# abelxiaoxing/ImageClassification

Hardware: AMD Instinct MI355X
Metric: images/sec (whole node) ResNet-50 bf16 224^2 training (higher is better)
Workload: dtype bf16; 1 GPU; resnet50 train step, synthetic 3x224x224, batch 256/GPU, AdamW, label smoothing 0.1, 1000 classes (BASELINE configs[1]); global_batch=256, parallelism=dp1

## Files before the change

imageclassification_amd/csrc/capi.hip:

```cpp
#include "../../include/icamd.h"
#include "common.h"
#include "icamd_internal.h"
#include <cstdlib>
#include <string.h>

int icamd_bn_finalize_launch(const float* part, int nrows, int C, double count, const float* gamma, const float* beta,
                             float* running_mean, float* running_var, float momentum, float eps, float* mean,
                             float* invstd, float* scale, float* shift, double* chunks, hipStream_t s);
int icamd_bn_eval_coeffs_launch(int C, const float* gamma, const float* beta, const float* rm, const float* rv, float eps,
                                float* scale, float* shift, hipStream_t s);
int icamd_bn_apply_launch(const bf16_t* y, const float* scale, const float* shift, const bf16_t* residual, bf16_t* out,
                          unsigned char* maskbits, long long numel, int C, int relu, hipStream_t s,
                          const float* res_scale = nullptr, const float* res_shift = nullptr);
int icamd_bn_bwd_rows_per_block(long long rows, int C);
int icamd_bn_bwd_launch(const bf16_t* dout, const bf16_t* act, const bf16_t* y, const float* mean, const float* invstd,
                        const float* scale, const float* shift, float* dgamma, float* dbeta, bf16_t* dy, bf16_t* gout,
                        const unsigned char* maskbits, long long rows, int C, int relu, int accumulate, float* part,
                        double* chunks, float* c1c2, hipStream_t s, const unsigned char* pool_idx = nullptr,
                        int pool_ih = 0, int pool_iw = 0);
int icamd_bn_bwd_dual_launch(const bf16_t* dout, const unsigned char* maskbits, const bf16_t* yA, const float* meanA,
                             const float* invstdA, const float* scaleA, float* dgammaA, float* dbetaA, bf16_t* dyA,
                             const bf16_t* yB, const float* meanB, const float* invstdB, const float* scaleB, float* dgammaB,
                             float* dbetaB, bf16_t* dyB, long long rows, int C, int accumulate, float* partA, double* chunksA,
                             float* cA, float* partB, double* chunksB, float* cB, hipStream_t s);
// ... 105 lines not shown
int icamd_se_bn_apply_launch(const bf16_t* y, const float* scale, const float* shift, const float* gate, const bf16_t* residual,
                             const float* res_scale, const float* res_shift, bf16_t* out, unsigned char* maskbits, int N, int HW,
                             int C, int relu, hipStream_t s);
size_t icamd_se_bn_bwd_bytes(int N, int HW, int C);
int icamd_se_bn_bwd_launch(const bf16_t* dout, const unsigned char* maskbits, const bf16_t* y, const float* mean,
                           const float* invstd, const float* gamma, const float* beta, const float* ysum, const float* sv,
                           const float* h, const float* e, const float* w1, const float* w2, float* dgamma, float* dbeta,
                           float* dw1, float* db1, float* dw2, float* db2, bf16_t* dy, int N, int HW, int C, int rd,
                           int accumulate, void* workspace, hipStream_t s);


#include <vector>
namespace {
enum ProfClass { PC_IGEMM_FWD = 0, PC_IGEMM_DGRAD, PC_WGRAD, PC_BN_FINALIZE, PC_BN_APPLY, PC_BN_BWD, PC_POOL, PC_PACK,
                 PC_LOSS, PC_OPTIM, PC_MISC, PC_ATTN_FWD, PC_ATTN_BWD, PC_LN_FWD, PC_LN_BWD, PC_ELEMWISE, PC_DWCONV, PC_FUSED_BWD, PC_FUSED_FWD, PC_COUNT };
struct ProfRec { int cls; hipEvent_t a, b; double bytes, flops; };
bool g_prof_on = false;
std::vector<ProfRec> g_prof_recs;
std::vector<hipEvent_t> g_prof_pool;
hipEvent_t prof_event() {
  if (!g_prof_pool.empty()) { hipEvent_t e = g_prof_pool.back(); g_prof_pool.pop_back(); return e; }
  hipEvent_t e; (void)hipEventCreate(&e); return e;
}
struct ProfScope {
  int cls; hipStream_t s; hipEvent_t a; bool on; double bytes = 0.0, flops = 0.0;
  ProfScope(int c, void* stream) : cls(c), s((hipStream_t)stream), on(g_prof_on) {
    if (on) { a = prof_event(); (void)hipEventRecord(a, s); }
  }
  void work(double b, double f = 0.0) { bytes = b; flops = f; }
  ~ProfScope() {
    if (on) { hipEvent_t b = prof_event(); (void)hipEventRecord(b, s); g_prof_recs.push_back({cls, a, b, bytes, flops}); }
  }
};
struct ConvWork { double in, out, w, flops; };
static ConvWork conv_work(const icamd_conv_desc* d) {
  ConvWork c = {0, 0, 0, 0};
  if (d == nullptr) return c;
  c.in = 2.0 * d->N * d->IH * d->IW * d->Cin;
  c.out = 2.0 * d->N * d->OH * d->OW * d->Cout;
  c.w = (double)d->Cout * d->KH * d->KW * d->Cin;
  c.flops = 2.0 * d->N * d->OH * d->OW * c.w;
  return c;
}
}

namespace {
// ... 14 lines not shown
}

extern "C" {

int icamd_abi_version(void) { return 6; }

int icamd_prof_enable(int on) { g_prof_on = on != 0; return ICAMD_OK; }
int icamd_prof_classes(void) { return PC_COUNT; }
int icamd_prof_collect(double* ms, long long* calls, double* bytes, double* flops, int n) {
  if (ms == nullptr || calls == nullptr || n < PC_COUNT) return ICAMD_ERR_BAD_ARG;
  for (auto& r : g_prof_recs) {
    (void)hipEventSynchronize(r.b);
    float t = 0.f;
    (void)hipEventElapsedTime(&t, r.a, r.b);
    ms[r.cls] += (double)t;
    calls[r.cls] += 1;
    if (bytes != nullptr) bytes[r.cls] += r.bytes;
    if (flops != nullptr) flops[r.cls] += r.flops;
    g_prof_pool.push_back(r.a);
    g_prof_pool.push_back(r.b);
  }
  g_prof_recs.clear();
  return ICAMD_OK;
}

int icamd_conv2d_stats_rows(const icamd_conv_desc* d) {
  if (!conv_desc_ok(d)) return 0;
  const long long M = (long long)d->N * d->OH * d->OW;
  return (int)((M + 127) / 128);
}

// ... 306 lines not shown
  int rc;
  if (dbias == nullptr && icamd_wgrad_halo_wanted(d->KH, d->KW, d->stride, d->pad, d->OH, d->OW, d->Cin, d->Cout, p.M)) {
    icamd_wgrad_halo_plan(p.M, p.Cin, p.Cout, &p.S, &p.rows_per_split);
    rc = icamd_wgrad_halo_launch(p, (hipStream_t)stream);
  } else {
    icamd_wgrad_plan(p.M, p.Cout, p.Ktot, &p.S, &p.rows_per_split);
    if (dbias != nullptr) p.bias_slab = p.slab + (size_t)p.S * p.Cout * p.Ktot;
    rc = icamd_wgrad_launch(p, (hipStream_t)stream);
  }
  if (rc) return rc;
  rc = icamd_slab_reduce_launch(p.slab, dw, (long long)p.Cout * p.Ktot, p.S, accumulate, (hipStream_t)stream);
  if (rc || dbias == nullptr) return rc;
  return icamd_slab_reduce_launch(p.bias_slab, dbias, (long long)p.Cout, p.S, accumulate, (hipStream_t)stream);
}

static bool gconv_ok(const icamd_conv_desc* d, int groups) {
  if (!conv_desc_ok(d) || groups <= 0) return false;
  if (d->KH != 3 || d->KW != 3 || d->pad != 1 || d->Cin != d->Cout) return false;
  return icamd_gconv3x3_ok(d->N, d->IH, d->IW, d->OH, d->OW, d->Cin, groups, d->stride);
}
static GConvParams gconv_params(const icamd_conv_desc* d, int groups) {
  GConvParams p;
  memset(&p, 0, sizeof(p));
  p.N = d->N; p.IH = d->IH; p.IW = d->IW; p.OH = d->OH; p.OW = d->OW; p.C = d->Cin; p.groups = groups; p.stride = d->stride;
  return p;
}
static void gconv_work(ProfScope& prof, const icamd_conv_desc* d, int groups, double filter_bytes_per_element) {
  if (d == nullptr || groups <= 0) return;
  const double wel = 9.0 * d->Cout * (d->Cin / groups);
  prof.work(2.0 * d->N * d->IH * d->IW * d->Cin + 2.0 * d->N * d->OH * d->OW * d->Cout + filter_bytes_per_element * wel,
// ... 1035 lines not shown
```

imageclassification_amd/csrc/conv_wgrad.hip:

```cpp
#include "common.h"
#include "icamd_internal.h"
#include <stdlib.h>

namespace {

constexpr int BKR = 64;

template <int W>
__device__ __forceinline__ int tr_swz(int row) {
  if constexpr (W >= 128) return (row & 3) | (((row >> 3) & 1) << 2);
  else return ((row >> 1) & 1) | (((row >> 3) & 1) << 1);
}

__device__ __forceinline__ bf16x8 tr_read_pair(const unsigned char* p0, const unsigned char* p1) {
  bf16x4 a = __builtin_amdgcn_ds_read_tr16_b64_v4i16((bf16x4 __attribute__((address_space(3)))*)p0);
  bf16x4 b = __builtin_amdgcn_ds_read_tr16_b64_v4i16((bf16x4 __attribute__((address_space(3)))*)p1);
  return bf16x8{a[0], a[1], a[2], a[3], b[0], b[1], b[2], b[3]};
}

__device__ __forceinline__ void wgrad_block_order(const WgradParams& p, unsigned int& tile, int& split) {
  const unsigned int nt = (unsigned)(p.ntiles_k * p.ntiles_c);
  if (p.xcd_chunk) {
    const unsigned int nblk = gridDim.x, xcd = blockIdx.x & 7u, idx = blockIdx.x >> 3;
    const unsigned int q = nblk >> 3, r = nblk & 7u;
// ... 4 lines not shown
  }
  const unsigned int grp = blockIdx.x / (8u * nt);
  const unsigned int rem = blockIdx.x - grp * 8u * nt;
  const unsigned int ns = min(8u, (unsigned)p.S - grp * 8u);
  tile = rem / ns;
  split = (int)(grp * 8u + (rem - tile * ns));
}

#ifndef ICAMD_WGRAD_STAGES
#define ICAMD_WGRAD_STAGES 1
#endif
#ifndef ICAMD_WGRAD_WAVES_PER_SIMD
#define ICAMD_WGRAD_WAVES_PER_SIMD 3
#endif

template <int BMK, int BNC>
__global__ __launch_bounds__(256, (ICAMD_WGRAD_STAGES == 1 ? ICAMD_WGRAD_WAVES_PER_SIMD : 2)) void conv_wgrad_kernel(const WgradParams p) {
  constexpr int NSTAGE = ICAMD_WGRAD_STAGES;
  constexpr int X_BYTES = BKR * BMK * 2;
  constexpr int Y_BYTES = BKR * BNC * 2;
  constexpr int STAGE_BYTES = X_BYTES + Y_BYTES;
  constexpr int XROWB = BMK * 2, YROWB = BNC * 2;
  constexpr int XCPR = BMK / 8, YCPR = BNC / 8;
  constexpr int XRPI = 64 / XCPR, YRPI = 64 / YCPR;
  constexpr int XJ = BMK / 32, YJ = BNC / 32;
  constexpr int KR = BMK / 32, CR = BNC / 32;
  __shared__ __attribute__((aligned(16))) unsigned char smem[NSTAGE * STAGE_BYTES];

  const int tid = threadIdx.x, lane = tid & 63, wave = tid >> 6;
  const int wk = wave & 1, wc = wave >> 1;

  unsigned int tile;
  int split;
  wgrad_block_order(p, tile, split);
  const int tile_c = (int)(tile % (unsigned)p.ntiles_c);
  const int tile_k = (int)(tile / (unsigned)p.ntiles_c);
  const int k0 = tile_k * BMK, c0 = tile_c * BNC;
  const int m_begin = split * p.rows_per_split;
  const int m_end = min(p.M, m_begin + p.rows_per_split);

  const bf16_t* __restrict__ x = p.x;
  const bf16_t* __restrict__ dy = p.dy;
  const bf16_t* zero = (const bf16_t*)icamd_zero_page;

  int x_row[XJ], x_dh[XJ], x_dw[XJ], x_ci[XJ];
#pragma unroll
  for (int j = 0; j < XJ; ++j) {
    const int row = (wave * XJ + j) * XRPI + lane / XCPR;
    const int pc = lane % XCPR;
// ... 508 lines not shown
      *(f32x4*)(slab + (long long)co * p.Ktot + kk) = acc[jj][ii];
    }
  if (do_bias && (lane >> 4) == 0) {
#pragma unroll
    for (int j = 0; j < 2; ++j) p.bias_slab[(long long)split * p.Cout + c0 + wc * 64 + wr * 32 + j * 16 + (lane & 15)] = bacc[j][0];
  }
}

#ifndef ICAMD_SLAB_NT
#define ICAMD_SLAB_NT 1
#endif
__device__ __forceinline__ f32x4 slab_ld(const f32x4* p) {
  if constexpr (ICAMD_SLAB_NT != 0) return __builtin_nontemporal_load(p);
  else return *p;
}
template <int OUTS>
__global__ __launch_bounds__(256) void slab_reduce_kernel(const float* __restrict__ slab, float* __restrict__ out,
                                                          long long n4, int S, int accumulate, int stem7_mask) {
  constexpr int LANES = 256 / OUTS;
  __shared__ f32x4 red[256];
  const int o = threadIdx.x % OUTS, l = threadIdx.x / OUTS;
  const long long i = (long long)blockIdx.x * OUTS + o;
  f32x4 a0 = {0.f, 0.f, 0.f, 0.f}, a1 = a0, a2 = a0, a3 = a0;
  if (i < n4) {
    const f32x4* p = (const f32x4*)slab + i;
    int k = l;
    for (; k + 3 * LANES < S; k += 4 * LANES) {
      a0 += slab_ld(p + (long long)k * n4);
      a1 += slab_ld(p + (long long)(k + LANES) * n4);
      a2 += slab_ld(p + (long long)(k + 2 * LANES) * n4);
      a3 += slab_ld(p + (long long)(k + 3 * LANES) * n4);
    }
    for (; k < S; k += LANES) a0 += slab_ld(p + (long long)k * n4);
  }
  red[threadIdx.x] = (a0 + a1) + (a2 + a3);
  __syncthreads();
  if (l == 0 && i < n4) {
// ... 311 lines not shown
  if (bmk == 256 && bnc == 256) return launch_ring<256, 256, 2, 4, 4, 2>(p, stream);
  if (bmk == 256 && bnc == 128) return launch_ring<256, 128, 2, 2, 3, 2>(p, stream);
  if (bmk == 128 && bnc == 256) return launch_ring<128, 256, 1, 4, 3, 2>(p, stream);
  if (bmk == 256 && bnc == 64) return launch_ring<256, 64, 4, 1, 3, 2>(p, stream);
  if (bmk == 64 && bnc == 256) return launch_ring<64, 256, 1, 4, 3, 2>(p, stream);
  if (bmk == 128 && bnc == 128) return launch_ring<128, 128, 2, 2, 3, 3>(p, stream);
  if (bmk == 128 && bnc == 64) return launch_ring<128, 64, 2, 2, 3, 3>(p, stream);
  if (bmk == 64 && bnc == 128) return launch_ring<64, 128, 2, 2, 3, 3>(p, stream);
  return launch_ring<64, 64, 2, 2, 3, 3>(p, stream);
}

int icamd_slab_reduce_launch(const float* slab, float* out, long long n, int S, int accumulate, hipStream_t stream,
                             int stem7_mask) {
  if (n % 4 != 0) return ICAMD_ERR_BAD_ARG;
  const long long n4 = n / 4;
  if (n4 >= 64 * 1024) {
    hipLaunchKernelGGL(slab_reduce_kernel<64>, dim3((unsigned)((n4 + 63) / 64)), dim3(256), 0, stream, slab, out, n4, S,
                       accumulate, stem7_mask);
  } else {
    hipLaunchKernelGGL(slab_reduce_kernel<16>, dim3((unsigned)((n4 + 15) / 16)), dim3(256), 0, stream, slab, out, n4, S,
                       accumulate, stem7_mask);
  }
  return icamd_launch_status();
}
```

imageclassification_amd/csrc/icamd_internal.h:

```cpp
#pragma once
#include "common.h"

#define ICAMD_MAX_TAPS 56

struct IgemmParams {
  const bf16_t* in;
  const bf16_t* wt;
  bf16_t* out;
  const bf16_t* addend;
  const unsigned char* addend_bits;
  int addend_sub2;
  const float* bias;
  float* stats;
  const bf16_t* bnb_y;
  const bf16_t* bnb_mask;
  const float *bnb_mean, *bnb_invstd, *bnb_scale, *bnb_shift;
  int bnb_relu;
  int relu;
  bf16_t* gelu_out;
  int gelu_inplace;
  const bf16_t* gelu_z;
  int N, IH, IW, Cin;
  int OH, OW, Cout;
  int P, Q, M;
// ... 193 lines not shown
  int S, rows_per_split;
  int ntiles_k, ntiles_c;
  int pointwise;
  int xcd_chunk;
  int stem7;
  FastDiv divHW, divW, divCin, divKW;
};
int icamd_wgrad_launch(WgradParams& p, hipStream_t stream);
void icamd_wgrad_plan(int M, int Cout, int Ktot, int* S, int* rows_per_split);
void icamd_wgrad_tile(long long M, int Ktot, int Cout, int* bmk, int* bnc);
bool icamd_wgrad_halo_wanted(int KH, int KW, int stride, int pad, int H, int W, int Cin, int Cout, long long M);
void icamd_wgrad_halo_plan(int M, int Cin, int Cout, int* S, int* rows_per_split);
int icamd_wgrad_halo_launch(WgradParams& p, hipStream_t stream);
int icamd_slab_reduce_launch(const float* slab, float* out, long long n, int S, int accumulate, hipStream_t stream,
                             int stem7_mask = 0);
```

imageclassification_amd/hip.py:

```python
import ctypes
import os
from ctypes import POINTER, Structure, c_double, c_float, c_int, c_longlong, c_size_t, c_void_p

import torch

_HERE = os.path.dirname(os.path.abspath(__file__))
LIB_PATH = os.path.join(_HERE, "csrc", "libicamd.so")

ABI_VERSION = 6
ERRORS = {1: "ICAMD_ERR_BAD_ARG", 2: "ICAMD_ERR_UNSUPPORTED", 3: "ICAMD_ERR_WORKSPACE", 4: "ICAMD_ERR_LAUNCH"}


class IcamdError(RuntimeError):
    pass


class BnBwdFuse(Structure):
    _fields_ = [("y", c_void_p), ("mask_src", c_void_p), ("mean", c_void_p), ("invstd", c_void_p), ("scale", c_void_p),
                ("shift", c_void_p), ("partials", c_void_p), ("relu", c_int)]


class ImageDesc(Structure):
    _fields_ = [("src_offset", ctypes.c_int64), ("src_h", c_int), ("src_w", c_int), ("crop_top", c_int), ("crop_left", c_int),
                ("crop_h", c_int), ("crop_w", c_int), ("hflip", c_int), ("vflip", c_int), ("jitter_order", c_int * 3),
# ... 37 lines not shown
    "icamd_conv2d_dgrad_sub2": (c_int, [POINTER(ConvDesc), _P, _P, _P, _P, _P]),
    "icamd_conv2d_dgrad_stats_rows": (c_int, [POINTER(ConvDesc)]),
    "icamd_conv2d_dgrad_bnbwd": (c_int, [POINTER(ConvDesc), _P, _P, _P, _P, POINTER(BnBwdFuse), _P]),
    "icamd_conv2d_dgrad_bnred_supported": (c_int, [POINTER(ConvDesc)]),
    "icamd_conv2d_dgrad_bnred": (c_int, [POINTER(ConvDesc), _P, _P, _P, _P, _P, c_int, _P, _P, _P, _P]),
    "icamd_bn_bwd_from_gy_partials": (c_int, [_P, c_int, _P, _P, _P, _P, _P, _P, _P, _P, c_longlong, c_int, c_int, _P, c_size_t, _P]),
    "icamd_bn_apply_conv1x1_fused_supported": (c_int, [POINTER(ConvDesc)]),
    "icamd_bn_apply_conv1x1_fused": (c_int, [POINTER(ConvDesc), _P, _P, _P, _P, _P, _P, _P, _P, _P, _P, _P, _P]),
    "icamd_conv1x1_bn_bwd_fused_supported": (c_int, [POINTER(ConvDesc)]),
    "icamd_conv1x1_bn_bwd_fused_workspace_bytes": (c_size_t, [POINTER(ConvDesc)]),
    "icamd_conv1x1_bn_bwd_fused": (c_int, [POINTER(ConvDesc), _P, c_int, _P, _P, _P, _P, _P, _P, _P, _P, _P, _P, _P, c_int, _P, c_size_t,
                                           _P, c_size_t, _P]),
    "icamd_conv2d_wgrad_workspace_bytes": (c_size_t, [POINTER(ConvDesc)]),
    "icamd_conv2d_wgrad": (c_int, [POINTER(ConvDesc), _P, _P, _P, c_int, _P, c_size_t, _P]),
    "icamd_conv2d_wgrad_bias": (c_int, [POINTER(ConvDesc), _P, _P, _P, _P, c_int, _P, c_size_t, _P]),
    "icamd_gconv3x3_supported": (c_int, [POINTER(ConvDesc), c_int]),
    "icamd_gconv3x3_fwd": (c_int, [POINTER(ConvDesc), c_int, _P, _P, _P, _P, _P]),
    "icamd_gconv3x3_fwd_act": (c_int, [POINTER(ConvDesc), c_int, _P, _P, _P, _P, c_int, _P]),
    "icamd_gconv3x3_dgrad": (c_int, [POINTER(ConvDesc), c_int, _P, _P, _P, _P]),
    "icamd_gconv3x3_wgrad_workspace_bytes": (c_size_t, [POINTER(ConvDesc), c_int]),
    "icamd_gconv3x3_wgrad": (c_int, [POINTER(ConvDesc), c_int, _P, _P, _P, c_int, _P, c_size_t, _P]),
    "icamd_avgpool2x2_fwd": (c_int, [_P, _P, c_int, c_int, c_int, c_int, _P]),
    "icamd_avgpool2x2_bwd": (c_int, [_P, _P, _P, c_int, c_int, c_int, c_int, _P]),
    "icamd_conv3x3_thin_supported": (c_int, [POINTER(ConvDesc)]),
    "icamd_conv3x3_thin_stats_rows": (c_int, [POINTER(ConvDesc)]),
    "icamd_conv3x3_thin_fwd": (c_int, [POINTER(ConvDesc), _P, _P, _P, _P, _P, c_int, _P]),
    "icamd_conv3x3_thin_dgrad": (c_int, [POINTER(ConvDesc), _P, _P, _P, _P]),
    "icamd_conv3x3_thin_wgrad_workspace_bytes": (c_size_t, [POINTER(ConvDesc)]),
    "icamd_conv3x3_thin_wgrad": (c_int, [POINTER(ConvDesc), _P, _P, _P, c_int, _P, c_size_t, _P]),
    "icamd_filter_transpose": (c_int, [_P, _P, _P, _P, c_int, _P]),
# ... 157 lines not shown
```

imageclassification_amd/nets.py:

```python
import ctypes
import itertools
import math
import os
from collections import OrderedDict
from types import SimpleNamespace

import torch

from . import hip
from .checkpoint import PicklableModel
from .streams import side_lane

BN_EPS = 1e-5
_FUSED_BNBWD = os.environ.get("ICAMD_FUSED_BNBWD", "0") == "1"
_WGRAD_STREAM = os.environ.get("ICAMD_WGRAD_STREAM", "1") != "0"
_DUAL_BNBWD = os.environ.get("ICAMD_DUAL_BNBWD", "1") != "0"
_SUB2_SHORTCUT = os.environ.get("ICAMD_SUB2_SHORTCUT", "1") != "0"
_FUSED_POOL_BWD = os.environ.get("ICAMD_FUSED_POOL_BWD", "1") != "0"
_STEM_THIN_DEFAULT = {"fwd": True, "dgrad": True, "wgrad": False}
_STEM_THIN_ENV = os.environ.get("ICAMD_STEM_THIN", "1")
_STEM_THIN = {op: (_STEM_THIN_ENV == "2" or (_STEM_THIN_ENV != "0" and on)) for op, on in _STEM_THIN_DEFAULT.items()}
BN_MOMENTUM = 0.1

ARCHS = {
    "resnet18": ("basic", [2, 2, 2, 2], 1, 64),
    "resnet34": ("basic", [3, 4, 6, 3], 1, 64),
    "resnet50": ("bottleneck", [3, 4, 6, 3], 1, 64),
    "resnet101": ("bottleneck", [3, 4, 23, 3], 1, 64),
    "resnet152": ("bottleneck", [3, 8, 36, 3], 1, 64),
    "wide_resnet50_2": ("bottleneck", [3, 4, 6, 3], 1, 128),
    "wide_resnet101_2": ("bottleneck", [3, 4, 23, 3], 1, 128),
    "resnext50_32x4d": ("bottleneck", [3, 4, 6, 3], 32, 4),
# ... 109 lines not shown

class _Conv:

    def __init__(self, name, cin, cout, k, stride, pad, cin_p=None, cout_p=None, bias=False, k_p=None, groups=1):
        self.name = name
        self.groups = groups
        self.cin, self.cout, self.k, self.stride, self.pad = cin, cout, k, stride, pad
        self.cin_p = cin_p or cin
        self.cout_p = cout_p or cout
        self.k_p = k_p or k
        self.has_bias = bias
        self.w = None
        self.b = None
        self.wt_offset = None
        self.descs = {}
        self.thin = False
        self.stem7 = False

    def desc(self, N, IH, IW):
        key = (N, IH, IW)
        d = self.descs.get(key)
        if d is None:
            d = hip.conv_desc(N, IH, IW, self.cin_p, self.cout_p, self.k, self.k, self.stride, self.pad)
            self.descs[key] = d
        return d


class _BN:
    def __init__(self, name, c):
        self.name, self.c = name, c
# ... 728 lines not shown
        return ws["logits"]

    def __call__(self, x_nchw):
        ws = self.pack(x_nchw.to(self.device, dtype=torch.float32).contiguous())
        logits = self.forward_packed(ws)
        return logits[:, : self.num_classes]

    def backward_packed(self, ws, accumulate=False):
        if _FUSED_BNBWD:
            if self.se:
                raise hip.IcamdError("ICAMD_FUSED_BNBWD=1 has no squeeze-and-excitation backward")
            if self.deep:
                raise hip.IcamdError("ICAMD_FUSED_BNBWD=1 has no average-pool shortcut backward")
            return self._backward_packed_fused(ws, accumulate)
        run = self._backward_begin(ws, accumulate, _WGRAD_STREAM and self.wgrad_side_stream)
        bufs = self._grad_buffers(ws)
        dout, other, run.T, run.DA = (b.data_ptr() for b in bufs[:4])
        run.ypool = itertools.cycle([b.data_ptr() for b in bufs[4:]])
        self._bwd_classifier(run, dout)
        fused_rows = 0
        for bi in range(len(self.blocks) - 1, -1, -1):
            dy, dy2, shortcut_done = self._bwd_last_bn(run, bi, dout, fused_rows)
            dy = self._bwd_inner_convs(run, bi, dy)
            fused_rows = self._bwd_conv1_shortcut(run, bi, dy, dy2, shortcut_done, dout, other)
            if run.hook:
                run.hook(self.blocks[bi]["convs"][0].w.offset, None, run.lane.events())
            dout, other = other, dout
        self._bwd_stem(run, dout, self._next_y(run), _FUSED_POOL_BWD)
        if run.hook:
            run.hook(0, None, run.lane.events())
        run.lane.join()

    def _backward_begin(self, ws, accumulate, side):
        lane = side_lane(self, "ICAMD_WGRAD_STREAM", True)
        lane.begin(side)
        return SimpleNamespace(ws=ws, N=ws["N"], acc=int(bool(accumulate)), lane=lane, s=lane.main.cuda_stream,
                               hook=self.grad_ready_hook, wsp=ws["wgrad_ws"].data_ptr(), wsb=ws["wgrad_ws_bytes"],
                               bws=ws["bnb_ws"].data_ptr(), bwb=ws["bnb_ws_bytes"])

    def _next_y(self, run):
        y = next(run.ypool)
        run.lane.before_write(y)
        return y

    def _side_wgrad(self, run, conv, d, x, dy):
        run.lane.launch(lambda st: self._wgrad(conv, d, x, dy, run.acc, run.wsp, run.wsb, st), reads=(dy,))

    def _bn_bwd(self, run, bn, dout, act, y, dy, gout, relu, maskbits=None):
        mean, invstd, scale, shift = self._stats(bn)
        c = bn.c
        hip.check(self.lib.icamd_bn_bwd(dout, act, y.data_ptr(), mean, invstd, scale, shift, self._gf(bn.weight),
                                        self._gf(bn.bias), dy, gout, maskbits, y.numel() // c, c, int(relu), run.acc, run.bws,
                                        run.bwb, run.s), bn.name + " bwd")

    def _fused_conv_bn(self, run, conv, bn, d, partials, nrows, g, y, x, dx, bn_ws, bn_ws_bytes):
        lib, ws = self.lib, run.ws
        mean, invstd, scale, _ = self._stats(bn)
        need = lib.icamd_conv1x1_bn_bwd_fused_workspace_bytes(ctypes.byref(d))
        fws = ws.get("fused_ws")
        if fws is None or fws.numel() < need:
            fws = ws["fused_ws"] = torch.empty(need, dtype=torch.uint8, device=self.device)
# ... 8 lines not shown
        dfc = self.fc.desc(N, 1, 1)
        self._side_wgrad(run, self.fc, dfc, ws["pooled"].data_ptr(), dl)
        hip.check(lib.icamd_colsum(dl, N, self.ncls_p, self.ncls_p, self._gf(self.fc.b), run.acc, s), "fc bias grad")
        self._dgrad(self.fc, dfc, dl, ws["dpooled"].data_ptr(), None, None, s)
        if run.hook:
            run.hook(self.fc.w.offset, self.n_params, run.lane.events())
        fh, fw = ws["final_hw"]
        hip.check(lib.icamd_avgpool_bwd(ws["dpooled"].data_ptr(), dout, N, fh * fw, self.feat_dim, s), "avgpool bwd")

    def _bwd_last_bn(self, run, bi, dout, fused_rows):
        lib, ws, N = self.lib, run.ws, run.N
        blk, b = self.blocks[bi], ws["blocks"][bi]
        conv3, bn3, y3 = blk["convs"][-1], blk["bns"][-1], b["y"][-1]
        down = "down_conv" in blk
        mask = b["mask"].data_ptr()
        dy = self._next_y(run)
        dy2, shortcut_done = None, False
        d3 = conv3.desc(N, *b["hw"][-1])
        if "se" in blk:
            se = blk["se"]
            mean, invstd, _, _ = self._stats(bn3)
            hip.check(lib.icamd_se_bn_bwd(dout, mask, y3.data_ptr(), mean, invstd, self._pf(bn3.weight), self._pf(bn3.bias),
                                          b["se_ysum"].data_ptr(), b["se_s"].data_ptr(), b["se_h"].data_ptr(),
                                          b["se_e"].data_ptr(), self._pf(se.w1), self._pf(se.w2), self._gf(bn3.weight),
                                          self._gf(bn3.bias), self._gf(se.w1), self._gf(se.b1), self._gf(se.w2), self._gf(se.b2),
                                          dy, N, d3.OH * d3.OW, se.c, se.rd, run.acc, ws["se_ws"].data_ptr(), ws["se_ws_bytes"],
                                          run.s), se.name + " + " + bn3.name + " bwd")
            return dy, None, False
        if (self.block == "bottleneck" and fused_rows > 0 and lib.icamd_conv1x1_bn_bwd_fused_supported(ctypes.byref(d3))):
            self._fused_conv_bn(run, conv3, bn3, d3, ws["bnb_part"].data_ptr(), fused_rows, dout, y3, b["a"][-2].data_ptr(), run.DA,
                                ws["bna_ws"].data_ptr(), ws["bna_ws_bytes"])
            dy = None
            if down:
                dc = blk["down_conv"]
                ddc = dc.desc(N, *b.get("short_hw", b["in_hw"]))
                if dc.stride == 1 and lib.icamd_conv1x1_bn_bwd_fused_supported(ctypes.byref(ddc)):
                    self._fused_conv_bn(run, dc, blk["down_bn"], ddc, None, 0, dout, b["yd"], b.get("xp", b["in"]).data_ptr(),
                                        run.T, run.bws, run.bwb)
                    shortcut_done = True
                else:
                    dy2 = self._next_y(run)
                    self._bn_bwd(run, blk["down_bn"], dout, None, b["yd"], dy2, None, False)
        elif down and _DUAL_BNBWD:
            dy2 = self._next_y(run)
            bnB = blk["down_bn"]
            meanA, invstdA, scaleA, _ = self._stats(bn3)
            meanB, invstdB, scaleB, _ = self._stats(bnB)
            c = bn3.c
            hip.check(lib.icamd_bn_bwd_dual(dout, mask, y3.data_ptr(), meanA, invstdA, scaleA, self._gf(bn3.weight),
                                            self._gf(bn3.bias), dy, b["yd"].data_ptr(), meanB, invstdB, scaleB,
                                            self._gf(bnB.weight), self._gf(bnB.bias), dy2, y3.numel() // c, c, run.acc, run.bws,
                                            ws["bnb_ws2"].data_ptr(), run.bwb, run.s), bn3.name + " + shortcut bwd")
        elif fused_rows:
            mean, invstd, scale, _ = self._stats(bn3)
            c = bn3.c
            hip.check(lib.icamd_bn_bwd_from_gy_partials(ws["bnb_part"].data_ptr(), fused_rows, dout, y3.data_ptr(), mean, invstd,
                                                        scale, self._gf(bn3.weight), self._gf(bn3.bias), dy, y3.numel() // c, c,
                                                        run.acc, ws["bna_ws"].data_ptr(), ws["bna_ws_bytes"], run.s),
                      bn3.name + " bwd (apply, sums from the data gradient)")
        else:
            self._bn_bwd(run, bn3, dout, None, y3, dy, None, True, mask)
        return dy, dy2, shortcut_done

    def _bwd_inner_convs(self, run, bi, dy):
        blk, b = self.blocks[bi], run.ws["blocks"][bi]
        convs, bns = blk["convs"], blk["bns"]
        for i in range(len(convs) - 1, 0, -1):
            if dy is not None:
                d = convs[i].desc(run.N, *b["hw"][i])
                self._side_wgrad(run, convs[i], d, b["a"][i - 1].data_ptr(), dy)
                self._dgrad(convs[i], d, dy, run.DA, None, None, run.s)
            dy = self._next_y(run)
            self._bn_bwd(run, bns[i - 1], run.DA, None, b["y"][i - 1], dy, None, True)
        return dy

    def _prev_takes_g(self, N, bi, h, w):
        if bi == 0 or self.block != "bottleneck":
            return False
        pblk = self.blocks[bi - 1]
        if "se" in pblk:
            return False
        if "down_conv" not in pblk:
            return True
        dp3 = pblk["convs"][-1].desc(N, h, w)
        return bool(self.lib.icamd_conv1x1_bn_bwd_fused_supported(ctypes.byref(dp3)))

    def _bwd_conv1_shortcut(self, run, bi, dy, dy2, shortcut_done, dout, other):
        lib, ws, N, s = self.lib, run.ws, run.N, run.s
        blk, b = self.blocks[bi], ws["blocks"][bi]
        conv1 = blk["convs"][0]
        h, w = b["in_hw"]
        xin = b["in"].data_ptr()
        d1 = conv1.desc(N, h, w)
        self._side_wgrad(run, conv1, d1, xin, dy)
        if blk.get("pool"):
            dc = blk["down_conv"]
            ddc = dc.desc(N, *b["short_hw"])
            if not shortcut_done:
                if dy2 is None:
                    dy2 = self._next_y(run)
                    self._bn_bwd(run, blk["down_bn"], dout, None, b["yd"], dy2, None, True, b["mask"].data_ptr())
                self._side_wgrad(run, dc, ddc, b["xp"].data_ptr(), dy2)
                self._dgrad(dc, ddc, dy2, run.T, None, None, s)
            self._dgrad(conv1, d1, dy, run.DA, None, None, s)
            hip.check(lib.icamd_avgpool2x2_bwd(run.T, run.DA, other, N, h, w, dc.cin_p, s), blk["name"] + " shortcut pool bwd")
            return 0
        if shortcut_done:
            self._dgrad(conv1, d1, dy, other, run.T, None, s)
            return 0
        if "down_conv" not in blk:
            addend, bits, on_even_grid = dout, b["mask"].data_ptr(), 0
        else:
            dc = blk["down_conv"]
            ddc = dc.desc(N, h, w)
            if dy2 is None:
                dy2 = self._next_y(run)
                self._bn_bwd(run, blk["down_bn"], dout, None, b["yd"], dy2, None, True, b["mask"].data_ptr())
            self._side_wgrad(run, dc, ddc, xin, dy2)
            if not (_SUB2_SHORTCUT and dc.k == 1 and dc.stride == 2 and dc.pad == 0):
                self._dgrad(dc, ddc, dy2, run.T, None, None, s)
                self._dgrad(conv1, d1, dy, other, run.T, None, s)
                return 0
            key = ("sub2", N, ddc.OH, ddc.OW)
            deven = dc.descs.get(key)
            if deven is None:
                deven = dc.descs[key] = hip.conv_desc(N, ddc.OH, ddc.OW, dc.cin_p, dc.cout_p, 1, 1, 1, 0)
            self._dgrad(dc, deven, dy2, run.T, None, None, s)
            addend, bits, on_even_grid = run.T, None, 1
        if self._prev_takes_g(N, bi, h, w) and lib.icamd_conv2d_dgrad_bnred_supported(ctypes.byref(d1)):
            pb = ws["blocks"][bi - 1]
            hip.check(lib.icamd_conv2d_dgrad_bnred(ctypes.byref(d1), dy, self._wt(conv1), other, addend, bits, on_even_grid,
# ... 110 lines not shown
```

include/icamd.h:

```cpp
#ifndef ICAMD_H
#define ICAMD_H
#include <stddef.h>
#include <stdint.h>

#ifdef __cplusplus
extern "C" {
#endif

#define ICAMD_OK 0
#define ICAMD_ERR_BAD_ARG 1
#define ICAMD_ERR_UNSUPPORTED 2
#define ICAMD_ERR_WORKSPACE 3
#define ICAMD_ERR_LAUNCH 4

int icamd_abi_version(void);

typedef struct icamd_conv_desc {
  int N, IH, IW, Cin;
  int OH, OW, Cout;
  int KH, KW, stride, pad;
} icamd_conv_desc;

int icamd_conv2d_stats_rows(const icamd_conv_desc* d);

// ... 19 lines not shown
  const void* y;
  const void* mask_src;
  const float *mean, *invstd, *scale, *shift;
  float* partials;
  int relu;
} icamd_bn_bwd_fuse;
int icamd_conv2d_dgrad_stats_rows(const icamd_conv_desc* d);
int icamd_conv2d_dgrad_bnbwd(const icamd_conv_desc* d, const void* dy, const void* w_t, void* g, const void* addend,
                             const icamd_bn_bwd_fuse* f, void* stream);

size_t icamd_conv2d_wgrad_workspace_bytes(const icamd_conv_desc* d);
int icamd_conv2d_wgrad(const icamd_conv_desc* d, const void* x, const void* dy, float* dw, int accumulate,
                       void* workspace, size_t workspace_bytes, void* stream);
int icamd_conv2d_wgrad_bias(const icamd_conv_desc* d, const void* x, const void* dy, float* dw, float* dbias,
                            int accumulate, void* workspace, size_t workspace_bytes, void* stream);

int icamd_gconv3x3_supported(const icamd_conv_desc* d, int groups);
int icamd_gconv3x3_fwd(const icamd_conv_desc* d, int groups, const void* x, const void* w, void* y, float* stats, void* stream);
int icamd_gconv3x3_fwd_act(const icamd_conv_desc* d, int groups, const void* x, const void* w, void* y, const float* bias, int relu,
                           void* stream);
int icamd_gconv3x3_dgrad(const icamd_conv_desc* d, int groups, const void* dy, const void* w, void* dx, void* stream);
size_t icamd_gconv3x3_wgrad_workspace_bytes(const icamd_conv_desc* d, int groups);
int icamd_gconv3x3_wgrad(const icamd_conv_desc* d, int groups, const void* x, const void* dy, float* dw, int accumulate,
                         void* workspace, size_t workspace_bytes, void* stream);

int icamd_filter_transpose(const void* src_base, void* dst_base, const int64_t* descs, const int32_t* jobs, int njobs,
                           void* stream);
int icamd_filter_transpose_tiled(const void* src_base, void* dst_base, const int64_t* descs, const int32_t* jobs,
                                 int njobs, void* stream);

// ... 247 lines not shown
```

Baseline: 14720 images/sec.

## Batch pointwise 1x1 weight-gradient convs into grouped wgrad and slab-reduce launches

Adds a grouped weight-gradient path that queues up to twelve 1x1 stride-1 convs with equal row counts and runs them as one multi-job GEMM kernel plus one grouped slab-reduce kernel on the side stream. Queued convs write their output gradients into dedicated held buffers so the data stays valid until the grouped launch. This targets launch overhead and under-filled grids from many small wgrad GEMMs. In exchange it uses extra memory for the held buffers and a larger workspace, and it delays gradient readiness, which changes when the hooks fire and how the work overlaps.

```diff
diff --git a/imageclassification_amd/csrc/capi.hip b/imageclassification_amd/csrc/capi.hip
--- a/imageclassification_amd/csrc/capi.hip
+++ b/imageclassification_amd/csrc/capi.hip
@@ -143,7 +143,7 @@
 namespace {
 enum ProfClass { PC_IGEMM_FWD = 0, PC_IGEMM_DGRAD, PC_WGRAD, PC_BN_FINALIZE, PC_BN_APPLY, PC_BN_BWD, PC_POOL, PC_PACK,
                  PC_LOSS, PC_OPTIM, PC_MISC, PC_ATTN_FWD, PC_ATTN_BWD, PC_LN_FWD, PC_LN_BWD, PC_ELEMWISE, PC_DWCONV, PC_FUSED_BWD, PC_FUSED_FWD, PC_COUNT };
-struct ProfRec { int cls; hipEvent_t a, b; double bytes, flops; };
+struct ProfRec { int cls; hipEvent_t a, b; double bytes, flops; int calls; };
 bool g_prof_on = false;
 std::vector<ProfRec> g_prof_recs;
 std::vector<hipEvent_t> g_prof_pool;
@@ -153,12 +153,13 @@
 }
 struct ProfScope {
   int cls; hipStream_t s; hipEvent_t a; bool on; double bytes = 0.0, flops = 0.0;
+  int calls = 1;
   ProfScope(int c, void* stream) : cls(c), s((hipStream_t)stream), on(g_prof_on) {
     if (on) { a = prof_event(); (void)hipEventRecord(a, s); }
   }
   void work(double b, double f = 0.0) { bytes = b; flops = f; }
   ~ProfScope() {
-    if (on) { hipEvent_t b = prof_event(); (void)hipEventRecord(b, s); g_prof_recs.push_back({cls, a, b, bytes, flops}); }
+    if (on) { hipEvent_t b = prof_event(); (void)hipEventRecord(b, s); g_prof_recs.push_back({cls, a, b, bytes, flops, calls}); }
   }
 };
 struct ConvWork { double in, out, w, flops; };
@@ -203,7 +204,7 @@
     float t = 0.f;
     (void)hipEventElapsedTime(&t, r.a, r.b);
     ms[r.cls] += (double)t;
-    calls[r.cls] += 1;
+    calls[r.cls] += r.calls;
     if (bytes != nullptr) bytes[r.cls] += r.bytes;
     if (flops != nullptr) flops[r.cls] += r.flops;
     g_prof_pool.push_back(r.a);
@@ -540,6 +541,62 @@
   return icamd_slab_reduce_launch(p.bias_slab, dbias, (long long)p.Cout, p.S, accumulate, (hipStream_t)stream);
 }
 
+int icamd_conv2d_wgrad_group_supported(const icamd_conv_desc* d) {
+  if (!conv_desc_ok(d)) return 0;
+  return icamd_wgrad_group_wanted(d->KH, d->KW, d->stride, d->pad, (long long)d->N * d->OH * d->OW, d->Cin, d->Cout) ? 1 : 0;
+}
+
+int icamd_conv2d_wgrad_group_plan(int n, const icamd_conv_desc* const* d, int* S, int* rows_per_split, unsigned int* first_block) {
+  if (n < 1 || n > ICAMD_WGRAD_GROUP_MAX || d == nullptr || S == nullptr || rows_per_split == nullptr || first_block == nullptr)
+    return ICAMD_ERR_BAD_ARG;
+  int M[ICAMD_WGRAD_GROUP_MAX], ci[ICAMD_WGRAD_GROUP_MAX], co[ICAMD_WGRAD_GROUP_MAX];
+  for (int j = 0; j < n; ++j) {
+    if (!icamd_conv2d_wgrad_group_supported(d[j])) return ICAMD_ERR_UNSUPPORTED;
+    M[j] = d[j]->N * d[j]->OH * d[j]->OW; ci[j] = d[j]->Cin; co[j] = d[j]->Cout;
+  }
+  icamd_wgrad_group_plan(n, M, ci, co, S, rows_per_split, first_block);
+  return ICAMD_OK;
+}
+
+size_t icamd_conv2d_wgrad_group_workspace_bytes(int n, const icamd_conv_desc* const* d) {
+  int S[ICAMD_WGRAD_GROUP_MAX], rows[ICAMD_WGRAD_GROUP_MAX];
+  unsigned int first[ICAMD_WGRAD_GROUP_MAX + 1];
+  if (icamd_conv2d_wgrad_group_plan(n, d, S, rows, first) != ICAMD_OK) return 0;
+  size_t bytes = 0;
+  for (int j = 0; j < n; ++j) bytes += (size_t)S[j] * d[j]->Cout * d[j]->Cin * sizeof(float);
+  return bytes;
+}
+
+int icamd_conv2d_wgrad_group(int n, const icamd_conv_desc* const* d, const void* const* x, const void* const* dy, float* const* dw,
+                             int accumulate, void* workspace, size_t workspace_bytes, void* stream) {
+  ProfScope _prof(PC_WGRAD, stream);
+  if (n < 1 || n > ICAMD_WGRAD_GROUP_MAX || d == nullptr || x == nullptr || dy == nullptr || dw == nullptr || workspace == nullptr)
+    return ICAMD_ERR_BAD_ARG;
+  int S[ICAMD_WGRAD_GROUP_MAX], rows[ICAMD_WGRAD_GROUP_MAX];
+  unsigned int first[ICAMD_WGRAD_GROUP_MAX + 1];
+  const int rc = icamd_conv2d_wgrad_group_plan(n, d, S, rows, first);
+  if (rc) return rc;
+  WgradGroupParams g;
+  memset(&g, 0, sizeof(g));
+  g.n = n;
+  double bytes = 0.0, flops = 0.0;
+  size_t off = 0;
+  for (int j = 0; j < n; ++j) {
+    if (x[j] == nullptr || dy[j] == nullptr || dw[j] == nullptr) return ICAMD_ERR_BAD_ARG;
+    const ConvWork cw = conv_work(d[j]);
+    bytes += cw.in + cw.out + 4 * cw.w; flops += cw.flops;
+    WgradGroupJob& jb = g.job[j];
+    jb.x = (const bf16_t*)x[j]; jb.dy = (const bf16_t*)dy[j]; jb.slab = (float*)((char*)workspace + off);
+    jb.M = d[j]->N * d[j]->OH * d[j]->OW; jb.Cin = d[j]->Cin; jb.Cout = d[j]->Cout;
+    jb.S = S[j]; jb.rows_per_split = rows[j];
+    off += (size_t)S[j] * jb.Cout * jb.Cin * sizeof(float);
+  }
+  _prof.work(bytes, flops);
+  _prof.calls = n;
+  if (workspace_bytes < off) return ICAMD_ERR_WORKSPACE;
+  return icamd_wgrad_group_launch(g, dw, accumulate, (hipStream_t)stream);
+}
+
 static bool gconv_ok(const icamd_conv_desc* d, int groups) {
   if (!conv_desc_ok(d) || groups <= 0) return false;
   if (d->KH != 3 || d->KW != 3 || d->pad != 1 || d->Cin != d->Cout) return false;
diff --git a/imageclassification_amd/csrc/conv_wgrad.hip b/imageclassification_amd/csrc/conv_wgrad.hip
--- a/imageclassification_amd/csrc/conv_wgrad.hip
+++ b/imageclassification_amd/csrc/conv_wgrad.hip
@@ -1,6 +1,7 @@
 #include "common.h"
 #include "icamd_internal.h"
 #include <stdlib.h>
+#include <string.h>
 
 namespace {
 
@@ -42,8 +43,57 @@
 #define ICAMD_WGRAD_WAVES_PER_SIMD 3
 #endif
 
-template <int BMK, int BNC>
-__global__ __launch_bounds__(256, (ICAMD_WGRAD_STAGES == 1 ? ICAMD_WGRAD_WAVES_PER_SIMD : 2)) void conv_wgrad_kernel(const WgradParams p) {
+template <class G>
+__device__ __forceinline__ int group_job_of(const G& g, unsigned int blk) {
+  int j = 0;
+#pragma unroll
+  for (int k = 1; k < ICAMD_WGRAD_GROUP_MAX; ++k) j += blk >= g.first[k] ? 1 : 0;
+  return j;
+}
+__device__ __forceinline__ WgradParams group_job_params(const WgradGroupParams& g, unsigned int& tile, int& split) {
+  unsigned int L = blockIdx.x;
+  if (g.xcd_chunk) {
+    const unsigned int nblk = gridDim.x, xcd = blockIdx.x & 7u, idx = blockIdx.x >> 3;
+    const unsigned int q = nblk >> 3, r = nblk & 7u;
+    L = (xcd < r ? xcd * (q + 1) : r * (q + 1) + (xcd - r) * q) + idx;
+  }
+  int j;
+  if (g.uniform_S > 0) {
+    const unsigned int S = (unsigned)g.uniform_S, T = gridDim.x / S;
+    const unsigned int s = L / T, rem = L - s * T;
+    j = group_job_of(g, rem * S);
+    tile = rem - g.first[j] / S;
+    split = (int)s;
+  } else {
+    j = group_job_of(g, L);
+  }
+  const WgradGroupJob& jb = g.job[j];
+  WgradParams p;
+  p.x = jb.x; p.dy = jb.dy; p.slab = jb.slab; p.bias_slab = nullptr;
+  p.N = 1; p.IH = 1; p.IW = jb.M; p.Cin = jb.Cin; p.OH = 1; p.OW = jb.M; p.Cout = jb.Cout;
+  p.KH = 1; p.KW = 1; p.stride = 1; p.pad = 0;
+  p.M = jb.M; p.Ktot = jb.Cin;
+  p.S = jb.S; p.rows_per_split = jb.rows_per_split;
+  p.ntiles_k = jb.ntiles_k; p.ntiles_c = jb.ntiles_c;
+  p.pointwise = 1; p.xcd_chunk = g.xcd_chunk; p.stem7 = 0;
+  p.divHW = FastDiv{0u, 0u, 1u, 0u}; p.divW = FastDiv{0u, 0u, 1u, 0u};
+  p.divCin = FastDiv{0u, 0u, 2u, 0u}; p.divKW = FastDiv{0u, 0u, 1u, 0u};
+  if (g.uniform_S <= 0) {
+    const unsigned int local = L - g.first[j], nt = (unsigned)(jb.ntiles_k * jb.ntiles_c);
+    split = (int)(local / nt);
+    tile = local - (unsigned)split * nt;
+  }
+  return p;
+}
+
+template <int BMK, int BNC, bool GROUPED = false>
+__global__ __launch_bounds__(256, (ICAMD_WGRAD_STAGES == 1 ? ICAMD_WGRAD_WAVES_PER_SIMD : 2)) void conv_wgrad_kernel(
+    const std::conditional_t<GROUPED, WgradGroupParams, WgradParams> arg) {
+  unsigned int tile;
+  int split;
+  WgradParams job;
+  if constexpr (GROUPED) job = group_job_params(arg, tile, split);
+  const WgradParams& p = [&]() -> const WgradParams& { if constexpr (GROUPED) return job; else return arg; }();
   constexpr int NSTAGE = ICAMD_WGRAD_STAGES;
   constexpr int X_BYTES = BKR * BMK * 2;
   constexpr int Y_BYTES = BKR * BNC * 2;
@@ -58,9 +108,7 @@
   const int tid = threadIdx.x, lane = tid & 63, wave = tid >> 6;
   const int wk = wave & 1, wc = wave >> 1;
 
-  unsigned int tile;
-  int split;
-  wgrad_block_order(p, tile, split);
+  if constexpr (!GROUPED) wgrad_block_order(p, tile, split);
   const int tile_c = (int)(tile % (unsigned)p.ntiles_c);
   const int tile_k = (int)(tile / (unsigned)p.ntiles_c);
   const int k0 = tile_k * BMK, c0 = tile_c * BNC;
@@ -599,13 +647,26 @@
   if constexpr (ICAMD_SLAB_NT != 0) return __builtin_nontemporal_load(p);
   else return *p;
 }
-template <int OUTS>
-__global__ __launch_bounds__(256) void slab_reduce_kernel(const float* __restrict__ slab, float* __restrict__ out,
-                                                          long long n4, int S, int accumulate, int stem7_mask) {
+struct SlabArgs { const float* slab; float* out; long long n4; int S, accumulate, stem7_mask; };
+template <int OUTS, bool GROUPED = false>
+__global__ __launch_bounds__(256) void slab_reduce_kernel(const std::conditional_t<GROUPED, SlabGroupParams, SlabArgs> arg) {
   constexpr int LANES = 256 / OUTS;
   __shared__ f32x4 red[256];
+  const float* __restrict__ slab;
+  float* __restrict__ out;
+  long long n4;
+  int S, accumulate, stem7_mask;
+  unsigned int bid = blockIdx.x;
+  if constexpr (GROUPED) {
+    const int j = group_job_of(arg, blockIdx.x);
+    const SlabGroupJob& jb = arg.job[j];
+    slab = jb.slab; out = jb.out; n4 = jb.n4; S = jb.S; accumulate = arg.accumulate; stem7_mask = 0;
+    bid = blockIdx.x - arg.first[j];
+  } else {
+    slab = arg.slab; out = arg.out; n4 = arg.n4; S = arg.S; accumulate = arg.accumulate; stem7_mask = arg.stem7_mask;
+  }
   const int o = threadIdx.x % OUTS, l = threadIdx.x / OUTS;
-  const long long i = (long long)blockIdx.x * OUTS + o;
+  const long long i = (long long)bid * OUTS + o;
   f32x4 a0 = {0.f, 0.f, 0.f, 0.f}, a1 = a0, a2 = a0, a3 = a0;
   if (i < n4) {
     const f32x4* p = (const f32x4*)slab + i;
@@ -947,12 +1008,80 @@
                              int stem7_mask) {
   if (n % 4 != 0) return ICAMD_ERR_BAD_ARG;
   const long long n4 = n / 4;
+  const SlabArgs a = {slab, out, n4, S, accumulate, stem7_mask};
   if (n4 >= 64 * 1024) {
-    hipLaunchKernelGGL(slab_reduce_kernel<64>, dim3((unsigned)((n4 + 63) / 64)), dim3(256), 0, stream, slab, out, n4, S,
-                       accumulate, stem7_mask);
+    hipLaunchKernelGGL(slab_reduce_kernel<64>, dim3((unsigned)((n4 + 63) / 64)), dim3(256), 0, stream, a);
   } else {
-    hipLaunchKernelGGL(slab_reduce_kernel<16>, dim3((unsigned)((n4 + 15) / 16)), dim3(256), 0, stream, slab, out, n4, S,
-                       accumulate, stem7_mask);
+    hipLaunchKernelGGL(slab_reduce_kernel<16>, dim3((unsigned)((n4 + 15) / 16)), dim3(256), 0, stream, a);
   }
   return icamd_launch_status();
 }
+
+bool icamd_wgrad_group_wanted(int KH, int KW, int stride, int pad, long long M, int Cin, int Cout) {
+  if (KH != 1 || KW != 1 || stride != 1 || pad != 0) return false;
+  if (M <= 0 || M >= (1ll << 30) || Cin <= 0 || Cout <= 0 || Cin % 8 != 0 || Cout % 8 != 0) return false;
+  if (M * Cin >= (1ll << 31)) return false;
+  int bmk, bnc;
+  icamd_wgrad_tile(M, Cin, Cout, &bmk, &bnc);
+  return bmk == 128 && bnc == 128 && !use_ring(bmk, bnc);
+}
+
+static constexpr int GROUP_GRID_FLOOR = 512;
+
+unsigned int icamd_wgrad_group_plan(int n, const int* M, const int* Cin, const int* Cout, int* S, int* rows_per_split,
+                                    unsigned int* first) {
+  long long tiles = 0;
+  for (int j = 0; j < n; ++j) tiles += (long long)((Cin[j] + 127) / 128) * ((Cout[j] + 127) / 128);
+  const long long want = tiles > 0 ? (GROUP_GRID_FLOOR + tiles - 1) / tiles : 1;
+  unsigned int blk = 0;
+  for (int j = 0; j < n; ++j) {
+    const int cap = (M[j] + BKR - 1) / BKR;
+    int s = (int)(want < cap ? want : cap);
+    if (s < 1) s = 1;
+    int r = (M[j] + s - 1) / s;
+    r = (r + BKR - 1) / BKR * BKR;
+    rows_per_split[j] = r;
+    S[j] = (M[j] + r - 1) / r;
+    first[j] = blk;
+    blk += (unsigned)(((Cin[j] + 127) / 128) * ((Cout[j] + 127) / 128) * S[j]);
+  }
+  first[n] = blk;
+  return blk;
+}
+
+int icamd_wgrad_group_launch(WgradGroupParams& g, float* const* dw, int accumulate, hipStream_t stream) {
+  if (g.n < 1 || g.n > ICAMD_WGRAD_GROUP_MAX) return ICAMD_ERR_BAD_ARG;
+  SlabGroupParams f;
+  memset(&f, 0, sizeof(f));
+  bool small = false;
+  unsigned int blk = 0;
+  for (int j = 0; j < g.n; ++j) {
+    WgradGroupJob& jb = g.job[j];
+    jb.ntiles_k = (jb.Cin + 127) / 128;
+    jb.ntiles_c = (jb.Cout + 127) / 128;
+    g.first[j] = blk;
+    blk += (unsigned)(jb.ntiles_k * jb.ntiles_c * jb.S);
+    f.job[j].slab = jb.slab; f.job[j].out = dw[j]; f.job[j].n4 = (long long)jb.Cout * jb.Cin / 4; f.job[j].S = jb.S;
+    if (f.job[j].n4 < 64 * 1024) small = true;
+  }
+  for (int j = g.n; j <= ICAMD_WGRAD_GROUP_MAX; ++j) g.first[j] = blk;
+  static const int xcd_chunk = [] { const char* e = getenv("ICAMD_WGRAD_XCD"); return (e ? atoi(e) : 1) && icamd_num_xccs() == 8; }();
+  g.xcd_chunk = xcd_chunk;
+  g.uniform_S = g.job[0].S;
+  for (int j = 1; j < g.n; ++j)
+    if (g.job[j].S != g.job[0].S) g.uniform_S = 0;
+  hipLaunchKernelGGL((conv_wgrad_kernel<128, 128, true>), dim3(blk), dim3(256), 0, stream, g);
+  int rc = icamd_launch_status();
+  if (rc) return rc;
+  const int outs = small ? 16 : 64;
+  unsigned int fblk = 0;
+  for (int j = 0; j < g.n; ++j) {
+    f.first[j] = fblk;
+    fblk += (unsigned)((f.job[j].n4 + outs - 1) / outs);
+  }
+  for (int j = g.n; j <= ICAMD_WGRAD_GROUP_MAX; ++j) f.first[j] = fblk;
+  f.n = g.n; f.accumulate = accumulate;
+  if (small) hipLaunchKernelGGL((slab_reduce_kernel<16, true>), dim3(fblk), dim3(256), 0, stream, f);
+  else hipLaunchKernelGGL((slab_reduce_kernel<64, true>), dim3(fblk), dim3(256), 0, stream, f);
+  return icamd_launch_status();
+}
diff --git a/imageclassification_amd/csrc/icamd_internal.h b/imageclassification_amd/csrc/icamd_internal.h
--- a/imageclassification_amd/csrc/icamd_internal.h
+++ b/imageclassification_amd/csrc/icamd_internal.h
@@ -231,3 +231,34 @@
 int icamd_wgrad_halo_launch(WgradParams& p, hipStream_t stream);
 int icamd_slab_reduce_launch(const float* slab, float* out, long long n, int S, int accumulate, hipStream_t stream,
                              int stem7_mask = 0);
+
+#define ICAMD_WGRAD_GROUP_MAX 12
+struct WgradGroupJob {
+  const bf16_t* x;
+  const bf16_t* dy;
+  float* slab;
+  int M, Cin, Cout;
+  int S, rows_per_split;
+  int ntiles_k, ntiles_c;
+};
+struct WgradGroupParams {
+  WgradGroupJob job[ICAMD_WGRAD_GROUP_MAX];
+  unsigned int first[ICAMD_WGRAD_GROUP_MAX + 1];
+  int n, xcd_chunk;
+  int uniform_S;
+};
+struct SlabGroupJob {
+  const float* slab;
+  float* out;
+  long long n4;
+  int S, pad;
+};
+struct SlabGroupParams {
+  SlabGroupJob job[ICAMD_WGRAD_GROUP_MAX];
+  unsigned int first[ICAMD_WGRAD_GROUP_MAX + 1];
+  int n, accumulate;
+};
+bool icamd_wgrad_group_wanted(int KH, int KW, int stride, int pad, long long M, int Cin, int Cout);
+unsigned int icamd_wgrad_group_plan(int n, const int* M, const int* Cin, const int* Cout, int* S, int* rows_per_split,
+                                    unsigned int* first);
+int icamd_wgrad_group_launch(WgradGroupParams& g, float* const* dw, int accumulate, hipStream_t stream);
diff --git a/imageclassification_amd/hip.py b/imageclassification_amd/hip.py
--- a/imageclassification_amd/hip.py
+++ b/imageclassification_amd/hip.py
@@ -75,6 +75,10 @@
     "icamd_conv2d_wgrad_workspace_bytes": (c_size_t, [POINTER(ConvDesc)]),
     "icamd_conv2d_wgrad": (c_int, [POINTER(ConvDesc), _P, _P, _P, c_int, _P, c_size_t, _P]),
     "icamd_conv2d_wgrad_bias": (c_int, [POINTER(ConvDesc), _P, _P, _P, _P, c_int, _P, c_size_t, _P]),
+    "icamd_conv2d_wgrad_group_supported": (c_int, [POINTER(ConvDesc)]),
+    "icamd_conv2d_wgrad_group_plan": (c_int, [c_int, _P, _P, _P, _P]),
+    "icamd_conv2d_wgrad_group_workspace_bytes": (c_size_t, [c_int, _P]),
+    "icamd_conv2d_wgrad_group": (c_int, [c_int, _P, _P, _P, _P, c_int, _P, c_size_t, _P]),
     "icamd_gconv3x3_supported": (c_int, [POINTER(ConvDesc), c_int]),
     "icamd_gconv3x3_fwd": (c_int, [POINTER(ConvDesc), c_int, _P, _P, _P, _P, _P]),
     "icamd_gconv3x3_fwd_act": (c_int, [POINTER(ConvDesc), c_int, _P, _P, _P, _P, c_int, _P]),
diff --git a/imageclassification_amd/nets.py b/imageclassification_amd/nets.py
--- a/imageclassification_amd/nets.py
+++ b/imageclassification_amd/nets.py
@@ -16,6 +16,8 @@
 _WGRAD_STREAM = os.environ.get("ICAMD_WGRAD_STREAM", "1") != "0"
 _DUAL_BNBWD = os.environ.get("ICAMD_DUAL_BNBWD", "1") != "0"
 _SUB2_SHORTCUT = os.environ.get("ICAMD_SUB2_SHORTCUT", "1") != "0"
+_WGRAD_GROUP = os.environ.get("ICAMD_WGRAD_GROUP", "1") != "0"
+_WGRAD_GROUP_MAX = 12
 _FUSED_POOL_BWD = os.environ.get("ICAMD_FUSED_POOL_BWD", "1") != "0"
 _STEM_THIN_DEFAULT = {"fwd": True, "dgrad": True, "wgrad": False}
 _STEM_THIN_ENV = os.environ.get("ICAMD_STEM_THIN", "1")
@@ -155,6 +157,7 @@
         self.b = None
         self.wt_offset = None
         self.descs = {}
+        self.grouped_wgrad = {}
         self.thin = False
         self.stem7 = False
 
@@ -913,6 +916,7 @@
                 raise hip.IcamdError("ICAMD_FUSED_BNBWD=1 has no average-pool shortcut backward")
             return self._backward_packed_fused(ws, accumulate)
         run = self._backward_begin(ws, accumulate, _WGRAD_STREAM and self.wgrad_side_stream)
+        run.group = _WGRAD_GROUP
         bufs = self._grad_buffers(ws)
         dout, other, run.T, run.DA = (b.data_ptr() for b in bufs[:4])
         run.ypool = itertools.cycle([b.data_ptr() for b in bufs[4:]])
@@ -922,8 +926,13 @@
             dy, dy2, shortcut_done = self._bwd_last_bn(run, bi, dout, fused_rows)
             dy = self._bwd_inner_convs(run, bi, dy)
             fused_rows = self._bwd_conv1_shortcut(run, bi, dy, dy2, shortcut_done, dout, other)
-            if run.hook:
-                run.hook(self.blocks[bi]["convs"][0].w.offset, None, run.lane.events())
+            lo = self.blocks[bi]["convs"][0].w.offset
+            if run.queue:
+                run.hook_lo = lo
+            elif run.hook:
+                run.hook(lo, None, run.lane.events())
+            if bi == 0 or self._stage(bi - 1) != self._stage(bi):
+                self._flush_wgrad_group(run)
             dout, other = other, dout
         self._bwd_stem(run, dout, self._next_y(run), _FUSED_POOL_BWD)
         if run.hook:
@@ -935,7 +944,7 @@
         lane.begin(side)
         return SimpleNamespace(ws=ws, N=ws["N"], acc=int(bool(accumulate)), lane=lane, s=lane.main.cuda_stream,
                                hook=self.grad_ready_hook, wsp=ws["wgrad_ws"].data_ptr(), wsb=ws["wgrad_ws_bytes"],
-                               bws=ws["bnb_ws"].data_ptr(), bwb=ws["bnb_ws_bytes"])
+                               bws=ws["bnb_ws"].data_ptr(), bwb=ws["bnb_ws_bytes"], group=False, queue=[], hook_lo=None)
 
     def _next_y(self, run):
         y = next(run.ypool)
@@ -943,7 +952,70 @@
         return y
 
     def _side_wgrad(self, run, conv, d, x, dy):
+        if self._wgrad_grouped(run, conv, d):
+            if dy != run.ws["wgrad_held"][conv.name].data_ptr():
+                raise hip.IcamdError(conv.name + ": a queued weight gradient must read its held output-gradient buffer")
+            if run.queue and self._rows(run.queue[0][1]) != self._rows(d):
+                self._flush_wgrad_group(run)
+            run.queue.append((conv, d, x, dy))
+            if len(run.queue) == _WGRAD_GROUP_MAX:
+                self._flush_wgrad_group(run)
+            return
         run.lane.launch(lambda st: self._wgrad(conv, d, x, dy, run.acc, run.wsp, run.wsb, st), reads=(dy,))
+
+    @staticmethod
+    def _rows(d):
+        return d.N * d.OH * d.OW
+
+    def _stage(self, bi):
+        return self.blocks[bi]["name"].split(".")[0]
+
+    def _wgrad_grouped(self, run, conv, d):
+        if not run.group or conv.stem7 or conv.groups > 1 or conv is self.fc:
+            return False
+        ok = conv.grouped_wgrad.get(d.key())
+        if ok is None:
+            ok = conv.grouped_wgrad[d.key()] = bool(self.lib.icamd_conv2d_wgrad_group_supported(ctypes.byref(d)))
+        return ok
+
+    def _dy_buffer(self, run, conv, d):
+        if not self._wgrad_grouped(run, conv, d):
+            return self._next_y(run)
+        held = run.ws.setdefault("wgrad_held", {})
+        buf = held.get(conv.name)
+        if buf is None:
+            buf = held[conv.name] = torch.empty(d.N * d.OH * d.OW * d.Cout, dtype=torch.bfloat16, device=self.device)
+        return buf.data_ptr()
+
+    def _flush_wgrad_group(self, run):
+        q, ws, lib = run.queue, run.ws, self.lib
+        if q:
+            run.queue = []
+            n = len(q)
+            key = tuple((conv.name, x, dy) for conv, _, x, dy in q)
+            args = ws.setdefault("wgrad_group_args", {}).get(key)
+            if args is None:
+                descs = (ctypes.POINTER(hip.ConvDesc) * n)(*[ctypes.pointer(d) for _, d, _, _ in q])
+                xs = (ctypes.c_void_p * n)(*[x for _, _, x, _ in q])
+                dys = (ctypes.c_void_p * n)(*[dy for _, _, _, dy in q])
+                dws = (ctypes.c_void_p * n)(*[self._gf(conv.w) for conv, _, _, _ in q])
+                need = lib.icamd_conv2d_wgrad_group_workspace_bytes(n, descs)
+                if need == 0:
+                    raise hip.IcamdError("no grouped weight gradient for " + ", ".join(c.name for c, _, _, _ in q))
+                args = ws["wgrad_group_args"][key] = (descs, xs, dys, dws, need)
+            descs, xs, dys, dws, need = args
+            if ws.get("wgrad_group_ws_bytes", 0) < need:
+                run.lane.join()
+                ws["wgrad_group_ws"] = torch.empty(need, dtype=torch.uint8, device=self.device)
+                ws["wgrad_group_ws_bytes"] = need
+            gws, gwb = ws["wgrad_group_ws"].data_ptr(), ws["wgrad_group_ws_bytes"]
+            run.lane.launch(lambda st: hip.check(lib.icamd_conv2d_wgrad_group(n, descs, xs, dys, dws, run.acc, gws, gwb, st),
+                                                 "grouped wgrad " + q[0][0].name + " .. " + q[-1][0].name),
+                            reads=tuple(dy for _, _, _, dy in q))
+        if run.hook_lo is not None:
+            if run.hook:
+                run.hook(run.hook_lo, None, run.lane.events())
+            run.hook_lo = None
 
     def _bn_bwd(self, run, bn, dout, act, y, dy, gout, relu, maskbits=None):
         mean, invstd, scale, shift = self._stats(bn)
@@ -982,9 +1054,11 @@
         conv3, bn3, y3 = blk["convs"][-1], blk["bns"][-1], b["y"][-1]
         down = "down_conv" in blk
         mask = b["mask"].data_ptr()
-        dy = self._next_y(run)
         dy2, shortcut_done = None, False
         d3 = conv3.desc(N, *b["hw"][-1])
+        fused = (self.block == "bottleneck" and "se" not in blk and fused_rows > 0
+                 and bool(lib.icamd_conv1x1_bn_bwd_fused_supported(ctypes.byref(d3))))
+        dy = self._next_y(run) if fused else self._dy_buffer(run, conv3, d3)
         if "se" in blk:
             se = blk["se"]
             mean, invstd, _, _ = self._stats(bn3)
@@ -995,7 +1069,7 @@
                                           dy, N, d3.OH * d3.OW, se.c, se.rd, run.acc, ws["se_ws"].data_ptr(), ws["se_ws_bytes"],
                                           run.s), se.name + " + " + bn3.name + " bwd")
             return dy, None, False
-        if (self.block == "bottleneck" and fused_rows > 0 and lib.icamd_conv1x1_bn_bwd_fused_supported(ctypes.byref(d3))):
+        if fused:
             self._fused_conv_bn(run, conv3, bn3, d3, ws["bnb_part"].data_ptr(), fused_rows, dout, y3, b["a"][-2].data_ptr(), run.DA,
                                 ws["bna_ws"].data_ptr(), ws["bna_ws_bytes"])
             dy = None
@@ -1007,10 +1081,10 @@
                                         run.T, run.bws, run.bwb)
                     shortcut_done = True
                 else:
-                    dy2 = self._next_y(run)
+                    dy2 = self._dy_buffer(run, dc, ddc)
                     self._bn_bwd(run, blk["down_bn"], dout, None, b["yd"], dy2, None, False)
         elif down and _DUAL_BNBWD:
-            dy2 = self._next_y(run)
+            dy2 = self._dy_buffer(run, blk["down_conv"], blk["down_conv"].desc(N, *b.get("short_hw", b["in_hw"])))
             bnB = blk["down_bn"]
             meanA, invstdA, scaleA, _ = self._stats(bn3)
             meanB, invstdB, scaleB, _ = self._stats(bnB)
@@ -1038,7 +1112,7 @@
                 d = convs[i].desc(run.N, *b["hw"][i])
                 self._side_wgrad(run, convs[i], d, b["a"][i - 1].data_ptr(), dy)
                 self._dgrad(convs[i], d, dy, run.DA, None, None, run.s)
-            dy = self._next_y(run)
+            dy = self._dy_buffer(run, convs[i - 1], convs[i - 1].desc(run.N, *b["hw"][i - 1]))
             self._bn_bwd(run, bns[i - 1], run.DA, None, b["y"][i - 1], dy, None, True)
         return dy
 
@@ -1066,7 +1140,7 @@
             ddc = dc.desc(N, *b["short_hw"])
             if not shortcut_done:
                 if dy2 is None:
-                    dy2 = self._next_y(run)
+                    dy2 = self._dy_buffer(run, dc, ddc)
                     self._bn_bwd(run, blk["down_bn"], dout, None, b["yd"], dy2, None, True, b["mask"].data_ptr())
                 self._side_wgrad(run, dc, ddc, b["xp"].data_ptr(), dy2)
                 self._dgrad(dc, ddc, dy2, run.T, None, None, s)
@@ -1082,7 +1156,7 @@
             dc = blk["down_conv"]
             ddc = dc.desc(N, h, w)
             if dy2 is None:
-                dy2 = self._next_y(run)
+                dy2 = self._dy_buffer(run, dc, ddc)
                 self._bn_bwd(run, blk["down_bn"], dout, None, b["yd"], dy2, None, True, b["mask"].data_ptr())
             self._side_wgrad(run, dc, ddc, xin, dy2)
             if not (_SUB2_SHORTCUT and dc.k == 1 and dc.stride == 2 and dc.pad == 0):
diff --git a/include/icamd.h b/include/icamd.h
--- a/include/icamd.h
+++ b/include/icamd.h
@@ -57,6 +57,11 @@
                        void* workspace, size_t workspace_bytes, void* stream);
 int icamd_conv2d_wgrad_bias(const icamd_conv_desc* d, const void* x, const void* dy, float* dw, float* dbias,
                             int accumulate, void* workspace, size_t workspace_bytes, void* stream);
+int icamd_conv2d_wgrad_group_supported(const icamd_conv_desc* d);
+int icamd_conv2d_wgrad_group_plan(int n, const icamd_conv_desc* const* d, int* S, int* rows_per_split, unsigned int* first_block);
+size_t icamd_conv2d_wgrad_group_workspace_bytes(int n, const icamd_conv_desc* const* d);
+int icamd_conv2d_wgrad_group(int n, const icamd_conv_desc* const* d, const void* const* x, const void* const* dy, float* const* dw,
+                             int accumulate, void* workspace, size_t workspace_bytes, void* stream);
 
 int icamd_gconv3x3_supported(const icamd_conv_desc* d, int groups);
 int icamd_gconv3x3_fwd(const icamd_conv_desc* d, int groups, const void* x, const void* w, void* y, float* stats, void* stream);
```

After: 14590 images/sec. About the same (-0.9%).
